# 1275468127/Medical-SAM2

Hardware: AMD Instinct MI355X
Metric: slices/sec @1024^2 (Hiera-S) (higher is better)
Workload: dtype bf16; 1 GPU; configs[1]: sam2_hiera_s 2D (train_2d SAM2 sub-sequence, forward), b=4 x 1024x1024 per GPU, 16-entry memory bank with 4 sampled memories per slice, one click per slice; forward_image -> memory_attention -> prompt encoder -> mask decoder -> memory encoder; hip_graph=True, weights=random name-keyed init

## Files before the change

### medical-sam2_amd/csrc/mlp_fused.hip

```cpp
#include "common.h"

struct MlpFusedParams {
  const float* x;
  float* out;
  const float *ln_w, *ln_b, *b1, *b2;
  const op16* w1;
  const op16* w2p;
  int64_t T;
  float eps;
  op16* out16;
};

template <int RB>
__device__ __forceinline__ int mlp_swz(int c, int r) {
  if constexpr (RB == 192) return (c & ~3) | ((c & 3) ^ ((r >> 2) & 3));
  else return (c & ~7) | ((c & 7) ^ ((r >> 1) & 7));
}

template <int DIM, int HC, int TB, int OCC = 1, int NWV = 4>
__global__ __launch_bounds__(NWV * 64, OCC) void mlp_fused_kernel(MlpFusedParams p) {
#if defined(__HIP_DEVICE_COMPILE__)
  constexpr int HID = 4 * DIM, NCH = HID / HC, KS1 = DIM / 16, DB = DIM / 32, HB = HC / 32;
  constexpr int RB1 = DIM * 2, RB2 = HC * 2;
  constexpr int CPR1 = DIM / 8, CPR2 = HC / 8;
  constexpr int W1B = HC * RB1, W2B = DIM * RB2, BUF = W1B + W2B;
  constexpr int PIECES1 = W1B / 1024, PIECES2 = W2B / 1024, PW1 = (PIECES1 + NWV - 1) / NWV, PW2 = (PIECES2 + NWV - 1) / NWV;
  static_assert((RB1 == 192 || RB1 == 384) && (RB2 == 192 || RB2 == 384), "row swizzles are built for 192 / 384-byte rows");
  static_assert(2 * BUF + (3 * DIM + HID) * 4 <= 160 * 1024, "LDS budget");
  extern __shared__ __attribute__((aligned(1024))) unsigned char smem[];
  float* prm = reinterpret_cast<float*>(smem + 2 * BUF);

  const int tid = threadIdx.x;
  const int wave = __builtin_amdgcn_readfirstlane(tid >> 6), lane = tid & 63;
  const int r = lane & 31, h = lane >> 5;
  for (int i = tid; i < DIM; i += NWV * 64) {
    prm[i] = p.ln_w[i];
    prm[DIM + i] = p.ln_b[i];
    prm[2 * DIM + i] = p.b2[i];
  }
  for (int i = tid; i < HID; i += NWV * 64) prm[3 * DIM + i] = p.b1[i];

  const auto w1_rsrc = raw_rsrc(p.w1, HID * DIM * 2);
  const auto w2_rsrc = raw_rsrc(p.w2p, HID * DIM * 2);
  unsigned off1[PW1], off2[PW2];
#pragma unroll
  for (int j = 0; j < PW1; ++j) {
    const int f = min(j * NWV + wave, PIECES1 - 1) * 64 + lane, row = f / CPR1, c = f % CPR1;
    off1[j] = (unsigned)(row * RB1 + mlp_swz<RB1>(c, row) * 16);
  }
#pragma unroll
  for (int j = 0; j < PW2; ++j) {
    const int f = min(j * NWV + wave, PIECES2 - 1) * 64 + lane, row = f / CPR2, c = f % CPR2;
    off2[j] = (unsigned)(row * HID * 2 + mlp_swz<RB2>(c, row) * 16);
  }
  auto issue = [&](int chunk, int buf) {
    unsigned char* d1 = smem + buf * BUF;
    unsigned char* d2 = smem + buf * BUF + W1B;
    const unsigned s1 = (unsigned)chunk * HC * RB1, s2 = (unsigned)chunk * HC * 2;
#pragma unroll
    for (int j = 0; j < PW1; ++j)
      if (j * NWV + wave < PIECES1)
        glds16(w1_rsrc, d1 + (j * NWV + wave) * 1024, off1[j], s1);
#pragma unroll
    for (int j = 0; j < PW2; ++j)
      if (j * NWV + wave < PIECES2)
        glds16(w2_rsrc, d2 + (j * NWV + wave) * 1024, off2[j], s2);
  };

  const int64_t pass_tokens = NWV * 32 * TB;
  const int64_t n_pass = (p.T + pass_tokens - 1) / pass_tokens;
  int64_t g_chunk = 0;
  constexpr bool RESIDENT = (NCH == 2) && NWV == 8;
  if ((int64_t)blockIdx.x < n_pass) {
    issue(0, 0);
    if constexpr (RESIDENT) issue(1, 1);
  }
  if constexpr (RESIDENT) wait_vmcnt<0>();
  __syncthreads();

  for (int64_t pass = blockIdx.x; pass < n_pass; pass += gridDim.x) {
    op16x8 xf[TB][KS1];
    int64_t tok[TB];
#pragma unroll
    for (int tb = 0; tb < TB; ++tb) {
      const int64_t t = pass * pass_tokens + (int64_t)(wave * TB + tb) * 32 + r;
      tok[tb] = t;
      const float* xr = p.x + (t < p.T ? t : p.T - 1) * DIM;
      f32x4 v[KS1][2];
      float s = 0.f;
#pragma unroll
      for (int k = 0; k < KS1; ++k)
#pragma unroll
        for (int q = 0; q < 2; ++q) {
          v[k][q] = *reinterpret_cast<const f32x4*>(xr + 16 * k + 8 * h + 4 * q);
          s += v[k][q][0] + v[k][q][1] + v[k][q][2] + v[k][q][3];
        }
      s += __shfl_xor(s, 32, 64);
      const float mean = s * (1.f / DIM);
      float q2 = 0.f;
#pragma unroll
      for (int k = 0; k < KS1; ++k)
#pragma unroll
        for (int q = 0; q < 2; ++q)
#pragma unroll
          for (int e = 0; e < 4; ++e) {
            const float dlt = v[k][q][e] - mean;
            q2 += dlt * dlt;
          }
      q2 += __shfl_xor(q2, 32, 64);
      const float rstd = 1.0f / sqrtf(q2 * (1.f / DIM) + p.eps);
#pragma unroll
      for (int k = 0; k < KS1; ++k) {
        op16x8 f;
#pragma unroll
        for (int q = 0; q < 2; ++q) {
          const f32x4 gm = *reinterpret_cast<const f32x4*>(prm + 16 * k + 8 * h + 4 * q);
          const f32x4 bt = *reinterpret_cast<const f32x4*>(prm + DIM + 16 * k + 8 * h + 4 * q);
#pragma unroll
          for (int e = 0; e < 4; ++e) f[4 * q + e] = f2op((v[k][q][e] - mean) * rstd * gm[e] + bt[e]);
        }
        xf[tb][k] = f;
      }
    }
    f32x16 accy[TB][DB];
#pragma unroll
    for (int tb = 0; tb < TB; ++tb)
#pragma unroll
      for (int d = 0; d < DB; ++d)
#pragma unroll
        for (int e = 0; e < 16; ++e) accy[tb][d][e] = 0.f;

    for (int chunk = 0; chunk < NCH; ++chunk, ++g_chunk) {
      const int buf = RESIDENT ? chunk : (int)(g_chunk & 1);
      if constexpr (!RESIDENT) {
        wait_vmcnt<0>();
        __builtin_amdgcn_s_barrier();
        const bool more_here = chunk + 1 < NCH;
        const bool more = more_here || (pass + gridDim.x < n_pass);
        if (more) issue(more_here ? chunk + 1 : 0, buf ^ 1);
      }
      const unsigned char* w1s = smem + buf * BUF;
      const unsigned char* w2s = w1s + W1B;
#pragma unroll 1
      for (int hb = 0; hb < HB; ++hb) {
        op16x8 a1[KS1];
        const int row1 = hb * 32 + r;
#pragma unroll
        for (int k = 0; k < KS1; ++k) a1[k] = *reinterpret_cast<const op16x8*>(w1s + row1 * RB1 + (mlp_swz<RB1>(2 * k + h, row1) << 4));
        f32x4 bias1[4];
#pragma unroll
        for (int g = 0; g < 4; ++g) bias1[g] = *reinterpret_cast<const f32x4*>(prm + 3 * DIM + chunk * HC + hb * 32 + 8 * g + 4 * h);
#pragma unroll
        for (int tb = 0; tb < TB; ++tb) {
          f32x16 acch;
#pragma unroll
          for (int e = 0; e < 16; ++e) acch[e] = bias1[e >> 2][e & 3];
#pragma unroll
          for (int k = 0; k < KS1; ++k) acch = MSAM2_MFMA_32x32x16(a1[k], xf[tb][k], acch, 0, 0, 0);
          op16x8 hf[2];
#pragma unroll
#ifdef MSAM2_MLP_NO_GELU
          for (int e = 0; e < 16; ++e) hf[e >> 3][e & 7] = f2op(acch[e]);
#else
          for (int e = 0; e < 16; e += 2) {
            const f32x2 gp = gelu_erf2(f32x2{acch[e], acch[e + 1]});
            hf[e >> 3][e & 7] = f2op(gp[0]);
            hf[e >> 3][(e & 7) + 1] = f2op(gp[1]);
          }
#endif
#pragma unroll
          for (int d = 0; d < DB; ++d) {
            const int row2 = d * 32 + r;
#pragma unroll
            for (int s2 = 0; s2 < 2; ++s2) {
              const op16x8 a2 = *reinterpret_cast<const op16x8*>(w2s + row2 * RB2 + (mlp_swz<RB2>(hb * 4 + 2 * s2 + h, row2) << 4));
              accy[tb][d] = MSAM2_MFMA_32x32x16(a2, hf[s2], accy[tb][d], 0, 0, 0);
            }
          }
        }
      }
    }
#pragma unroll
    for (int tb = 0; tb < TB; ++tb) {
      if (tok[tb] < p.T) {
        const float* xr = p.x + tok[tb] * DIM;
        float* yr = p.out + tok[tb] * DIM;
        constexpr int DG = 1;
        static_assert(DB % DG == 0, "d-blocks in whole batches");
#pragma unroll
        for (int d0 = 0; d0 < DB; d0 += DG) {
          f32x4 xv[DG][4];
#pragma unroll
          for (int d = 0; d < DG; ++d)
#pragma unroll
            for (int g = 0; g < 4; ++g) xv[d][g] = *reinterpret_cast<const f32x4*>(xr + (d0 + d) * 32 + 8 * g + 4 * h);
#pragma unroll
          for (int d = 0; d < DG; ++d)
#pragma unroll
            for (int g = 0; g < 4; ++g) {
              const int ch = (d0 + d) * 32 + 8 * g + 4 * h;
              const f32x4 bv = *reinterpret_cast<const f32x4*>(prm + 2 * DIM + ch);
              f32x4 o;
#pragma unroll
              for (int e = 0; e < 4; ++e) o[e] = accy[tb][d0 + d][4 * g + e] + bv[e] + xv[d][g][e];
              *reinterpret_cast<f32x4*>(yr + ch) = o;
              if (p.out16) {
                op16x4 o2;
#pragma unroll
                for (int e = 0; e < 4; ++e) o2[e] = f2op(o[e]);
                *reinterpret_cast<op16x4*>(p.out16 + tok[tb] * DIM + ch) = o2;
              }
            }
        }
      }
    }
  }
#endif
}

__device__ __forceinline__ int mlp_swz768(int c, int r) { return (c & ~15) | ((c & 15) ^ (r & 15)); }

__global__ __launch_bounds__(256, 1) void mlp_fused384_kernel(MlpFusedParams p) {
#if defined(__HIP_DEVICE_COMPILE__)
  constexpr int DIM = 384, HID = 1536, HC = 32, NCH = HID / HC, KS1 = DIM / 16, DBW = 6, NST = 3;
  constexpr int W1B = HC * DIM * 2, W2B = DIM * HC * 2, BUF = W1B + W2B;
  constexpr int PW = W1B / 1024 / 4;
  static_assert(NST * BUF + (3 * DIM + HID) * 4 <= 160 * 1024, "LDS budget");
  extern __shared__ __attribute__((aligned(1024))) unsigned char smem[];
  float* prm = reinterpret_cast<float*>(smem + NST * BUF);

  const int tid = threadIdx.x;
  const int wave = __builtin_amdgcn_readfirstlane(tid >> 6), lane = tid & 63;
  const int r = lane & 31, h = lane >> 5;
  const int tb = wave >> 1, dh = wave & 1;
  for (int i = tid; i < DIM; i += 256) {
    prm[i] = p.ln_w[i];
    prm[DIM + i] = p.ln_b[i];
    prm[2 * DIM + i] = p.b2[i];
  }
  for (int i = tid; i < HID; i += 256) prm[3 * DIM + i] = p.b1[i];

  const int64_t t = (int64_t)blockIdx.x * 64 + tb * 32 + r;
  const float* xr = p.x + (t < p.T ? t : p.T - 1) * DIM;
  f32x4 v[KS1][2];
#pragma unroll
  for (int k = 0; k < KS1; ++k)
#pragma unroll
    for (int q = 0; q < 2; ++q) v[k][q] = *reinterpret_cast<const f32x4*>(xr + 16 * k + 8 * h + 4 * q);

  const auto w1_rsrc = raw_rsrc(p.w1, HID * DIM * 2);
  const auto w2_rsrc = raw_rsrc(p.w2p, HID * DIM * 2);
  unsigned off1[PW];
#pragma unroll
  for (int j = 0; j < PW; ++j) {
    const int f = (j * 4 + wave) * 64 + lane, row = f / 48, c = f % 48;
    off1[j] = (unsigned)(row * 768 + mlp_swz768(c, row) * 16);
  }
  const unsigned off2 = (unsigned)(wave * 1024 + lane * 16);
  auto issue = [&](int i) {
    unsigned char* d1 = smem + (i % NST) * BUF;
    unsigned char* d2 = d1 + W1B;
    if (i < NCH) {
      const unsigned s = (unsigned)i * W1B;
#pragma unroll
      for (int j = 0; j < PW; ++j)
        glds16(w1_rsrc, d1 + (j * 4 + wave) * 1024, off1[j], s);
    }
    if (i >= 1) {
      const unsigned s = (unsigned)(i - 1) * W2B;
#pragma unroll
      for (int j = 0; j < PW; ++j)
        glds16(w2_rsrc, d2 + (j * 4 + wave) * 1024, off2, s + j * 4096);
    }
  };
  issue(0);
  issue(1);

  op16x8 xf[KS1];
  {
    float s = 0.f;
#pragma unroll
    for (int k = 0; k < KS1; ++k)
#pragma unroll
      for (int q = 0; q < 2; ++q) s += v[k][q][0] + v[k][q][1] + v[k][q][2] + v[k][q][3];
    s += __shfl_xor(s, 32, 64);
    const float mean = s * (1.f / DIM);
    float q2 = 0.f;
#pragma unroll
    for (int k = 0; k < KS1; ++k)
#pragma unroll
      for (int q = 0; q < 2; ++q)
#pragma unroll
        for (int e = 0; e < 4; ++e) {
          const float dlt = v[k][q][e] - mean;
          q2 += dlt * dlt;
        }
    q2 += __shfl_xor(q2, 32, 64);
    const float rstd = 1.0f / sqrtf(q2 * (1.f / DIM) + p.eps);
    __builtin_amdgcn_s_waitcnt(0xc07f);
    __builtin_amdgcn_s_barrier();
    asm volatile("" ::: "memory");
#pragma unroll
    for (int k = 0; k < KS1; ++k) {
      op16x8 f;
#pragma unroll
      for (int q = 0; q < 2; ++q) {
        const f32x4 gm = *reinterpret_cast<const f32x4*>(prm + 16 * k + 8 * h + 4 * q);
        const f32x4 bt = *reinterpret_cast<const f32x4*>(prm + DIM + 16 * k + 8 * h + 4 * q);
#pragma unroll
        for (int e = 0; e < 4; ++e) f[4 * q + e] = f2op((v[k][q][e] - mean) * rstd * gm[e] + bt[e]);
      }
      xf[k] = f;
    }
  }
  f32x16 accy[DBW];
#pragma unroll
  for (int d = 0; d < DBW; ++d)
#pragma unroll
    for (int e = 0; e < 16; ++e) accy[d][e] = 0.f;

  auto fc1_gelu = [&](const unsigned char* w1s, int chunk, f32x16& acch, const f32x16* aprev, op16x8 (&hf)[2]) {
    op16x8 fa[8], fb[8];
    auto rd = [&](op16x8 (&f)[8], int k0) {
#pragma unroll
      for (int k = 0; k < 8; ++k) f[k] = *reinterpret_cast<const op16x8*>(w1s + r * 768 + (mlp_swz768(2 * (k0 + k) + h, r) << 4));
    };
    rd(fa, 0);
    rd(fb, 8);
    f32x4 bias1[4];
#pragma unroll
    for (int g = 0; g < 4; ++g) bias1[g] = *reinterpret_cast<const f32x4*>(prm + 3 * DIM + chunk * HC + 8 * g + 4 * h);
    f32x16 part[2];
#pragma unroll
    for (int e = 0; e < 16; ++e) {
      part[0][e] = bias1[e >> 2][e & 3];
      part[1][e] = 0.f;
    }
    __builtin_amdgcn_sched_barrier(0);
#pragma unroll
    for (int k = 0; k < 8; ++k) part[k & 1] = MSAM2_MFMA_32x32x16(fa[k], xf[k], part[k & 1], 0, 0, 0);
    if (aprev) {
#pragma unroll
      for (int e = 0; e < 6; e += 2) {
        const f32x2 gp = gelu_erf2(f32x2{(*aprev)[e], (*aprev)[e + 1]});
        hf[e >> 3][e & 7] = f2op(gp[0]);
        hf[e >> 3][(e & 7) + 1] = f2op(gp[1]);
      }
    }
#pragma unroll
    for (int q = 0; q < 8; ++q) {
      __builtin_amdgcn_sched_group_barrier(0x008, 1, 0);
      __builtin_amdgcn_sched_group_barrier(0x002, 6, 0);
    }
    __builtin_amdgcn_sched_barrier(0);
    rd(fa, 16);
#pragma unroll
    for (int k = 0; k < 8; ++k) part[k & 1] = MSAM2_MFMA_32x32x16(fb[k], xf[8 + k], part[k & 1], 0, 0, 0);
    if (aprev) {
#pragma unroll
      for (int e = 6; e < 12; e += 2) {
        const f32x2 gp = gelu_erf2(f32x2{(*aprev)[e], (*aprev)[e + 1]});
        hf[e >> 3][e & 7] = f2op(gp[0]);
        hf[e >> 3][(e & 7) + 1] = f2op(gp[1]);
      }
    }
#pragma unroll
    for (int q = 0; q < 8; ++q) {
      __builtin_amdgcn_sched_group_barrier(0x008, 1, 1);
      __builtin_amdgcn_sched_group_barrier(0x002, 6, 1);
    }
    __builtin_amdgcn_sched_barrier(0);
#pragma unroll
    for (int k = 0; k < 8; ++k) part[k & 1] = MSAM2_MFMA_32x32x16(fa[k], xf[16 + k], part[k & 1], 0, 0, 0);
    if (aprev) {
#pragma unroll
      for (int e = 12; e < 16; e += 2) {
        const f32x2 gp = gelu_erf2(f32x2{(*aprev)[e], (*aprev)[e + 1]});
        hf[e >> 3][e & 7] = f2op(gp[0]);
        hf[e >> 3][(e & 7) + 1] = f2op(gp[1]);
      }
    }
#pragma unroll
    for (int q = 0; q < 8; ++q) {
      __builtin_amdgcn_sched_group_barrier(0x008, 1, 2);
      __builtin_amdgcn_sched_group_barrier(0x002, 5, 2);
    }
    __builtin_amdgcn_sched_barrier(0);
#pragma unroll
    for (int e = 0; e < 16; ++e) acch[e] = part[0][e] + part[1][e];
  };
  auto gelu16 = [&](const f32x16& acch, op16x8 (&hf)[2]) {
#pragma unroll
    for (int e = 0; e < 16; e += 2) {
      const f32x2 gp = gelu_erf2(f32x2{acch[e], acch[e + 1]});
      hf[e >> 3][e & 7] = f2op(gp[0]);
      hf[e >> 3][(e & 7) + 1] = f2op(gp[1]);
    }
  };
  auto fc2 = [&](const unsigned char* w2s, const op16x8 (&hf)[2]) {
    op16x8 a2[DBW][2];
#pragma unroll
    for (int d = 0; d < DBW; ++d) {
      const int row2 = (dh * DBW + d) * 32 + r;
#pragma unroll
      for (int s2 = 0; s2 < 2; ++s2) a2[d][s2] = *reinterpret_cast<const op16x8*>(w2s + row2 * Img64::ROW_BYTES + (((2 * s2 + h) ^ Img64::swz(row2)) << 4));
    }
#pragma unroll
    for (int s2 = 0; s2 < 2; ++s2)
#pragma unroll
      for (int d = 0; d < DBW; ++d) accy[d] = MSAM2_MFMA_32x32x16(a2[d][s2], hf[s2], accy[d], 0, 0, 0);
  };

  f32x16 acur;
  wait_vmcnt<12>();
  __builtin_amdgcn_s_barrier();
  issue(2);
  {
    op16x8 hf0[2];
    fc1_gelu(smem, 0, acur, nullptr, hf0);
  }
#pragma unroll 1
  for (int i = 1; i < NCH; ++i) {
    if (i + 1 < NCH) wait_vmcnt<12>();
    else wait_vmcnt<6>();
    __builtin_amdgcn_s_barrier();
    if (i + 2 <= NCH) issue(i + 2);
    const unsigned char* w1s = smem + (i % NST) * BUF;
    f32x16 anext;
    op16x8 hf[2];
    fc1_gelu(w1s, i, anext, &acur, hf);
    fc2(w1s + W1B, hf);
    acur = anext;
  }
  {
    wait_vmcnt<0>();
    __builtin_amdgcn_s_barrier();
    op16x8 hf[2];
    gelu16(acur, hf);
    fc2(smem + (NCH % NST) * BUF + W1B, hf);
  }

  if (t < p.T) {
    const float* xres = p.x + t * DIM;
    float* yr = p.out + t * DIM;
    constexpr int DG = 3;
#pragma unroll
    for (int d0 = 0; d0 < DBW; d0 += DG) {
      f32x4 xv[DG][4];
#pragma unroll
      for (int d = 0; d < DG; ++d)
#pragma unroll
        for (int g = 0; g < 4; ++g) xv[d][g] = *reinterpret_cast<const f32x4*>(xres + (dh * DBW + d0 + d) * 32 + 8 * g + 4 * h);
#pragma unroll
      for (int d = 0; d < DG; ++d)
#pragma unroll
        for (int g = 0; g < 4; ++g) {
          const int ch = (dh * DBW + d0 + d) * 32 + 8 * g + 4 * h;
          const f32x4 bv = *reinterpret_cast<const f32x4*>(prm + 2 * DIM + ch);
          f32x4 o;
#pragma unroll
          for (int e = 0; e < 4; ++e) o[e] = accy[d0 + d][4 * g + e] + bv[e] + xv[d][g][e];
          *reinterpret_cast<f32x4*>(yr + ch) = o;
          if (p.out16) {
            op16x4 o2;
#pragma unroll
            for (int e = 0; e < 4; ++e) o2[e] = f2op(o[e]);
            *reinterpret_cast<op16x4*>(p.out16 + t * DIM + ch) = o2;
          }
        }
    }
  }
#endif
}

__global__ void mlp_fused384_pack_kernel(const op16* __restrict__ w2, op16* __restrict__ w2q, int dim, int hid) {
  const int64_t total = (int64_t)dim * hid;
  for (int64_t i = (int64_t)blockIdx.x * blockDim.x + threadIdx.x; i < total; i += (int64_t)gridDim.x * blockDim.x) {
    const int chunk = (int)(i / ((int64_t)dim * 32)), d = (int)((i / 32) % dim), q = (int)(i & 31);
    const int c = (q >> 3) ^ Img64::swz(d), j = q & 7, pos = c * 8 + j;
    const int s = pos >> 4, hh = (pos >> 3) & 1;
    w2q[i] = w2[(int64_t)d * hid + chunk * 32 + 16 * s + 8 * (j >> 2) + 4 * hh + (j & 3)];
  }
}

__global__ void mlp_fused_permute_kernel(const op16* __restrict__ w2, op16* __restrict__ w2p, int dim, int hid) {
  const int64_t total = (int64_t)dim * hid;
  for (int64_t i = (int64_t)blockIdx.x * blockDim.x + threadIdx.x; i < total; i += (int64_t)gridDim.x * blockDim.x) {
    const int d = (int)(i / hid), pos = (int)(i % hid);
    const int blk = pos >> 5, q = pos & 31, s = q >> 4, hh = (q >> 3) & 1, j = q & 7;
    w2p[i] = w2[(int64_t)d * hid + blk * 32 + 16 * s + 8 * (j >> 2) + 4 * hh + (j & 3)];
  }
}

extern "C" int msam2_mlp_fused_permute_w2(const void* w2, void* w2p, int64_t dim, int64_t hidden, void* stream) {
  MSAM2_REQUIRE(w2 && w2p && dim > 0 && hidden % 32 == 0, "mlp_fused_permute_w2: bad arguments");
  if (dim == 384) {
    MSAM2_REQUIRE(hidden == 1536, "mlp_fused_permute_w2: dim 384 takes hidden 1536");
    hipLaunchKernelGGL(mlp_fused384_pack_kernel, dim3(1024), dim3(256), 0, (hipStream_t)stream, (const op16*)w2, (op16*)w2p, (int)dim, (int)hidden);
    return msam2_check_launch("mlp_fused_permute_w2(384)");
  }
  hipLaunchKernelGGL(mlp_fused_permute_kernel, dim3((unsigned)min((int64_t)1024, cdiv(dim * hidden, 256))), dim3(256), 0, (hipStream_t)stream,
                     (const op16*)w2, (op16*)w2p, (int)dim, (int)hidden);
  return msam2_check_launch("mlp_fused_permute_w2");
}

extern "C" int msam2_ln_mlp_residual_supported(int64_t dim) {
  static const bool use384 = [] { const char* e = getenv("MSAM2_MLP_384"); return e && e[0] == '1'; }();
  return dim == 96 || dim == 192 || (dim == 384 && use384);
}

static int launch_mlp_fused384(const MlpFusedParams& p, hipStream_t s) {
  constexpr int LDS = 3 * 49152 + (3 * 384 + 1536) * 4;
  ensure_dyn_lds<mlp_fused384_kernel>(LDS);
  hipLaunchKernelGGL(mlp_fused384_kernel, dim3((unsigned)((p.T + 63) / 64)), dim3(256), LDS, s, p);
  return msam2_check_launch("ln_mlp_residual_fwd(384)");
}

template <int DIM, int HC, int TB, int OCC = 1, int NWV = 4>
static int launch_mlp_fused(const MlpFusedParams& p, hipStream_t s) {
  constexpr int LDS = 2 * (2 * HC * DIM * 2) + (3 * DIM + 4 * DIM) * 4;
  ensure_dyn_lds<mlp_fused_kernel<DIM, HC, TB, OCC, NWV>>(LDS);
  const int64_t n_pass = (p.T + NWV * 32 * TB - 1) / (NWV * 32 * TB);
  hipLaunchKernelGGL((mlp_fused_kernel<DIM, HC, TB, OCC, NWV>), dim3((unsigned)min((int64_t)256 * OCC, n_pass)), dim3(NWV * 64), LDS, s, p);
  return msam2_check_launch("ln_mlp_residual_fwd");
}

static int ln_mlp_residual_launch(const float* x, int64_t T, int64_t dim, const float* ln_w, const float* ln_b, float eps, const void* w1,
                                  const float* b1, const void* w2p, const float* b2, float* out, void* out16, void* stream) {
  MSAM2_REQUIRE(x && out && ln_w && ln_b && w1 && b1 && w2p && b2 && T > 0, "ln_mlp_residual: null tensor / empty problem");
  MSAM2_REQUIRE(dim == 96 || dim == 192 || dim == 384, "ln_mlp_residual: dim %lld not built (96 / 192 / 384)", (long long)dim);
  MSAM2_REQUIRE((((uintptr_t)x | (uintptr_t)out | (uintptr_t)w1 | (uintptr_t)w2p | (uintptr_t)ln_w | (uintptr_t)ln_b | (uintptr_t)b1 | (uintptr_t)b2) & 15) == 0 &&
                    ((uintptr_t)out16 & 7) == 0, "ln_mlp_residual: 16-byte aligned tensors");
  MSAM2_REQUIRE(x != out, "ln_mlp_residual: in-place not supported (a token's residual is re-read in the store)");
  MlpFusedParams p = {x, out, ln_w, ln_b, b1, b2, (const op16*)w1, (const op16*)w2p, T, eps, (op16*)out16};
  hipStream_t s = (hipStream_t)stream;
  if (dim == 384) {
    MSAM2_REQUIRE((T + 63) / 64 < (1ll << 31), "ln_mlp_residual: too many tokens");
    return launch_mlp_fused384(p, s);
  }
  static const bool four = [] { const char* e = getenv("MSAM2_MLP_WAVES4"); return e && e[0] == '1'; }();
  if (four) {
    if (dim == 96) return launch_mlp_fused<96, 192, 4>(p, s);
    return launch_mlp_fused<192, 96, 2>(p, s);
  }
  if (dim == 96) return launch_mlp_fused<96, 192, 2, 1, 8>(p, s);
  return launch_mlp_fused<192, 96, 1, 1, 8>(p, s);
}

extern "C" int msam2_ln_mlp_residual_fwd(const float* x, int64_t T, int64_t dim, const float* ln_w, const float* ln_b, float eps, const void* w1,
                                         const float* b1, const void* w2p, const float* b2, float* out, void* stream) {
  return ln_mlp_residual_launch(x, T, dim, ln_w, ln_b, eps, w1, b1, w2p, b2, out, nullptr, stream);
}

extern "C" int msam2_ln_mlp_residual_fwd_dual(const float* x, int64_t T, int64_t dim, const float* ln_w, const float* ln_b, float eps,
                                              const void* w1, const float* b1, const void* w2p, const float* b2, float* out, void* out16,
                                              void* stream) {
  MSAM2_REQUIRE(out16, "ln_mlp_residual_dual: null 16-bit output");
  return ln_mlp_residual_launch(x, T, dim, ln_w, ln_b, eps, w1, b1, w2p, b2, out, out16, stream);
}
```

### medical-sam2_amd/ops.py

```python
from __future__ import annotations

import ctypes
import math
from typing import Optional, Tuple

import torch

from ._lib import check, lib

OP16 = torch.float16 if lib().msam2_operand_is_fp16() else torch.bfloat16

F32 = torch.float32
ACT_NONE, ACT_GELU, ACT_RELU, ACT_SIGMOID = 0, 1, 2, 3


def _stream() -> int:
    return torch.cuda.current_stream().cuda_stream


def _p(t: Optional[torch.Tensor]):
    return None if t is None else t.data_ptr()


def _is_bf16(t: torch.Tensor) -> int:
    if t.dtype == OP16:
        return 1
    if t.dtype == F32:
        return 0
    raise TypeError(f"expected {OP16} or fp32 tensor, got {t.dtype}")


def _req(cond: bool, msg: str):
    if not cond:
        raise ValueError(msg)


def gemm(a: torch.Tensor, w: torch.Tensor, bias: Optional[torch.Tensor] = None, *, act: int = ACT_NONE,
         colscale: Optional[torch.Tensor] = None, residual: Optional[torch.Tensor] = None, res_mod: int = 0,
         out_dtype: torch.dtype = OP16, out: Optional[torch.Tensor] = None) -> torch.Tensor:
    _req(a.dim() == 2 and w.dim() == 2 and a.shape[1] == w.shape[1], f"gemm shapes {tuple(a.shape)} x {tuple(w.shape)}")
    _req(a.dtype == OP16 and w.dtype == OP16, "gemm operands must be 16-bit (ops.OP16)")
    _req(a.stride(1) == 1 and w.stride(1) == 1, "gemm operands must be K-contiguous")
    M, K = a.shape
    N = w.shape[0]
    if out is None:
        out = torch.empty(M, N, dtype=out_dtype, device=a.device)
    _req(out.stride(1) == 1 and out.shape == (M, N), "gemm out must be [M,N] row-major")
    if residual is not None:
        _req(residual.dim() == 2 and residual.stride(1) == 1 and residual.shape[1] == N, "gemm residual must be [*,N]")
    check(lib().msam2_gemm(_p(a), a.stride(0), _p(w), w.stride(0), _p(bias), _p(colscale), _p(residual),
                                residual.stride(0) if residual is not None else 0,
                                _is_bf16(residual) if residual is not None else 0, res_mod, _p(out), out.stride(0),
                                _is_bf16(out), M, N, K, act, _stream()))
    return out


def gemm_tokens(a: torch.Tensor, w: torch.Tensor, bias: Optional[torch.Tensor] = None, *, addend: Optional[torch.Tensor] = None,
                add_cols: int = 0, act: int = ACT_NONE, residual: Optional[torch.Tensor] = None, out_dtype: torch.dtype = OP16) -> torch.Tensor:
    _req(a.dim() == 2 and a.dtype == F32 and a.stride(1) == 1 and a.shape[0] <= 32, "gemm_tokens: a must be fp32 [M<=32, K]")
    _req(w.dtype == OP16 and w.stride(1) == 1 and w.shape[1] == a.shape[1], "gemm_tokens: w must be 16-bit [N, K]")
    if addend is not None:
        _req(addend.dtype == F32 and addend.shape == a.shape and addend.stride(1) == 1 and addend.stride(0) == a.stride(0),
             "gemm_tokens: addend must match a")
    M, K = a.shape
    N = w.shape[0]
    out = torch.empty(M, N, dtype=out_dtype, device=a.device)
    if residual is not None:
        _req(residual.dtype == F32 and residual.shape == (M, N) and residual.stride(1) == 1, "gemm_tokens: residual must be fp32 [M,N]")
    check(lib().msam2_gemm_tokens(_p(a), a.stride(0), _p(addend), add_cols if addend is not None else 0, _p(w), w.stride(0), _p(bias),
                                  _p(residual), residual.stride(0) if residual is not None else 0, _p(out), out.stride(0), _is_bf16(out),
                                  M, N, K, act, _stream()))
    return out


def gemm_pool2x2(a: torch.Tensor, w: torch.Tensor, bias: Optional[torch.Tensor], B: int, H: int, W: int) -> torch.Tensor:
    _req(a.dim() == 2 and w.dim() == 2 and a.shape[1] == w.shape[1] and a.shape[0] == B * H * W, "gemm_pool2x2 shapes")
    _req(a.dtype == OP16 and w.dtype == OP16 and a.stride(1) == 1 and w.stride(1) == 1, "gemm_pool2x2 operands: 16-bit, K-contiguous")
    N, K = w.shape
    out = torch.empty(B * (H // 2) * (W // 2), N, dtype=F32, device=a.device)
    check(lib().msam2_gemm_pool2x2(_p(a), a.stride(0), _p(w), w.stride(0), _p(bias), _p(out), out.stride(0), B, H, W, N, K, _stream()))
    return out


def gemm_qkv_pool2x2(a: torch.Tensor, w: torch.Tensor, bias: Optional[torch.Tensor], B: int, H: int, W: int, q_cols: int):
    _req(a.dim() == 2 and w.dim() == 2 and a.shape[1] == w.shape[1] and a.shape[0] == B * H * W, "gemm_qkv_pool2x2 shapes")
    _req(a.dtype == OP16 and w.dtype == OP16 and a.stride(1) == 1 and w.stride(1) == 1, "gemm_qkv_pool2x2 operands: 16-bit, K-contiguous")
    N, K = w.shape
    qkv = torch.empty(B * H * W, N, dtype=OP16, device=a.device)
    q2 = torch.empty(B * (H // 2) * (W // 2), q_cols, dtype=OP16, device=a.device)
    check(lib().msam2_gemm_qkv_pool2x2(_p(a), a.stride(0), _p(w), w.stride(0), _p(bias), _p(qkv), qkv.stride(0), _p(q2), q2.stride(0),
                                       B, H, W, N, K, q_cols, _stream()))
    return qkv, q2


def gemm_rope(a: torch.Tensor, w: torch.Tensor, bias: Optional[torch.Tensor], table: Tuple[torch.Tensor, torch.Tensor], *,
              rope_cols: int, head_dim: int, rows_per_batch: int, n_rope: int, out: Optional[torch.Tensor] = None) -> torch.Tensor:
    _req(a.dim() == 2 and w.dim() == 2 and a.shape[1] == w.shape[1], f"gemm_rope shapes {tuple(a.shape)} x {tuple(w.shape)}")
    _req(a.dtype == OP16 and w.dtype == OP16 and a.stride(1) == 1 and w.stride(1) == 1, "gemm_rope operands: 16-bit, K-contiguous")
    cs, sn = table
    _req(cs.dtype == F32 and cs.is_contiguous() and sn.is_contiguous() and cs.shape == sn.shape and cs.shape[1] * 2 == head_dim,
         "gemm_rope: table must be cos/sin fp32 [n_pos, head_dim/2]")
    M, K = a.shape
    N = w.shape[0]
    if out is None:
        out = torch.empty(M, N, dtype=OP16, device=a.device)
    _req(out.dtype == OP16 and out.shape == (M, N) and out.stride(1) == 1, "gemm_rope: out must be 16-bit [M, N] row-major")
    check(lib().msam2_gemm_rope(_p(a), a.stride(0), _p(w), w.stride(0), _p(bias), _p(out), out.stride(0), M, N, K, _p(cs), _p(sn),
                                rope_cols, head_dim, rows_per_batch, n_rope, cs.shape[0], _stream()))
    return out


def layernorm(x: torch.Tensor, weight: torch.Tensor, bias: torch.Tensor, eps: float, *, act: int = ACT_NONE,
              out_dtype: torch.dtype = OP16) -> torch.Tensor:
    C = x.shape[-1]
    x2 = x.reshape(-1, C)
    _req(x2.stride(1) == 1, "layernorm input rows must be contiguous")
    y = torch.empty(x2.shape, dtype=out_dtype, device=x.device)
    check(lib().msam2_layernorm(_p(x2), _is_bf16(x2), x2.stride(0), _p(weight), _p(bias), _p(y), _is_bf16(y), y.stride(0),
                                x2.shape[0], C, eps, act, _stream()))
    return y.reshape(x.shape)


def layernorm_dual(x: torch.Tensor, weight: torch.Tensor, bias: torch.Tensor, eps: float):
    C = x.shape[-1]
    x2 = x.reshape(-1, C)
    _req(x2.dtype == F32 and x2.stride(1) == 1 and C % 4 == 0, "layernorm_dual: fp32 rows, C % 4 == 0")
    y = torch.empty(x2.shape, dtype=F32, device=x.device)
    y16 = torch.empty(x2.shape, dtype=OP16, device=x.device)
    check(lib().msam2_layernorm_dual(_p(x2), x2.stride(0), _p(weight), _p(bias), _p(y), y.stride(0), _p(y16), y16.stride(0), x2.shape[0], C, eps,
                                     _stream()))
    return y.reshape(x.shape), y16.reshape(x.shape)


def ln_mlp_residual_supported(dim: int) -> bool:
    return bool(lib().msam2_ln_mlp_residual_supported(dim))


def mlp_fused_permute_w2(w2: torch.Tensor) -> torch.Tensor:
    _req(w2.dim() == 2 and w2.dtype == OP16 and w2.is_contiguous() and w2.shape[1] % 32 == 0, "mlp_fused_permute_w2: 16-bit [dim, hidden]")
    out = torch.empty_like(w2)
    check(lib().msam2_mlp_fused_permute_w2(_p(w2), _p(out), w2.shape[0], w2.shape[1], _stream()))
    return out


def ln_mlp_residual(x: torch.Tensor, ln_w: torch.Tensor, ln_b: torch.Tensor, eps: float, w1: torch.Tensor, b1: torch.Tensor, w2p: torch.Tensor,
                    b2: torch.Tensor, also16: bool = False):
    T, dim = x.shape
    _req(x.dtype == F32 and x.is_contiguous() and w1.dtype == OP16 and w2p.dtype == OP16 and w1.shape == (4 * dim, dim) and w2p.shape == (dim, 4 * dim)
         and w1.is_contiguous() and w2p.is_contiguous(), "ln_mlp_residual: x fp32 [T, dim], w1 [4 dim, dim], w2p [dim, 4 dim] 16-bit contiguous")
    out = torch.empty_like(x)
    if also16:
        out16 = torch.empty(x.shape, dtype=OP16, device=x.device)
        check(lib().msam2_ln_mlp_residual_fwd_dual(_p(x), T, dim, _p(ln_w), _p(ln_b), float(eps), _p(w1), _p(b1), _p(w2p), _p(b2), _p(out), _p(out16),
                                                   _stream()))
        return out, out16
    check(lib().msam2_ln_mlp_residual_fwd(_p(x), T, dim, _p(ln_w), _p(ln_b), float(eps), _p(w1), _p(b1), _p(w2p), _p(b2), _p(out), _stream()))
    return out


def _strides3(t: torch.Tensor) -> "ctypes.Array":
    return (ctypes.c_int64 * 3)(t.stride(0), t.stride(1), t.stride(2))


def attention(q: torch.Tensor, k: torch.Tensor, v: torch.Tensor, *, splits: int = 1,
              out: Optional[torch.Tensor] = None, scale: Optional[float] = None, workspace: Optional[torch.Tensor] = None,
              defer_merge: bool = False, lse: Optional[torch.Tensor] = None, dropout: Optional[tuple] = None) -> torch.Tensor:
    B, H, Lq, D = q.shape
    Lk = k.shape[2]
    for t in (q, k, v):
        _req(t.dtype == OP16 and t.stride(3) == 1, "attention tensors must be 16-bit (ops.OP16) with contiguous head dim")
    if out is None:
        out = torch.empty(B, Lq, H, D, dtype=OP16, device=q.device).permute(0, 2, 1, 3)
    if lse is not None:
        _req(lse.dtype == F32 and lse.is_contiguous() and lse.numel() == B * H * Lq and not defer_merge, "attention: lse must be fp32 [B,H,Lq]")
        splits = max(splits, 2)
    ws_bytes = lib().msam2_attention_workspace_bytes(B, H, Lq, D, splits)
    ws = workspace if workspace is not None else (torch.empty(max(ws_bytes, 1), dtype=torch.uint8, device=q.device) if splits > 1 else None)
    _req(not defer_merge or (workspace is not None and splits > 1), "defer_merge needs splits > 1 and a caller-owned workspace")
    _req(ws is None or ws.numel() * ws.element_size() >= ws_bytes, "attention workspace too small")
    sc = scale if scale is not None else 1.0 / math.sqrt(D)
    if dropout is not None and dropout[0] > 0:
        _req(lse is not None, "attention: dropout is a training feature (pass lse)")
        pd, seed, offset = dropout
        seed_dev = None
        if isinstance(seed, DeviceSeed):
            seed, seed_dev = seed.base, seed.dev
        check(lib().msam2_attention_fwd_lse_dropout(_p(q), _strides3(q), _p(k), _strides3(k), _p(v), _strides3(v), _p(out), _strides3(out),
                                                    B, H, Lq, Lk, D, sc, splits, _p(ws), ws_bytes if ws is not None else 0, _p(lse), float(pd),
                                                    int(seed) & (2 ** 64 - 1), int(offset) & (2 ** 64 - 1), _p(seed_dev), _stream()))
        return out
    if lse is not None:
        check(lib().msam2_attention_fwd_lse(_p(q), _strides3(q), _p(k), _strides3(k), _p(v), _strides3(v), _p(out), _strides3(out),
                                            B, H, Lq, Lk, D, sc, splits, _p(ws), ws_bytes if ws is not None else 0, _p(lse), _stream()))
        return out
    check(lib().msam2_attention_fwd(_p(q), _strides3(q), _p(k), _strides3(k), _p(v), _strides3(v), _p(out), _strides3(out),
                                    B, H, Lq, Lk, D, sc, -splits if defer_merge else splits, _p(ws), ws_bytes if ws is not None else 0, _stream()))
    return out


def attention_kv64(q: torch.Tensor, k: torch.Tensor, v: torch.Tensor, *, splits: int = 1, scale: Optional[float] = None,
                   workspace: Optional[torch.Tensor] = None, defer_merge: bool = False,
                   key_count: Optional[torch.Tensor] = None, out: Optional[torch.Tensor] = None) -> torch.Tensor:
    B, H, Lq, D = q.shape
    Lk = k.shape[2]
    _req(D == 256 and k.shape[3] == 256 and v.shape[3] == 64 and v.shape[2] == Lk, "attention_kv64: q/k rows of 256, v rows of 64")
    _req(key_count is None or (key_count.dtype == torch.int32 and key_count.numel() == 1 and key_count.device == q.device),
         "attention_kv64: key_count is one int32 on the tensors' device")
    for t in (q, k, v):
        _req(t.dtype == OP16 and t.stride(3) == 1, "attention tensors must be 16-bit (ops.OP16) with contiguous head dim")
    if out is None:
        out = torch.empty(B, Lq, H, 64, dtype=OP16, device=q.device).permute(0, 2, 1, 3)
    _req(out.dtype == OP16 and out.shape == (B, H, Lq, 64) and out.stride(3) == 1, "attention_kv64: out is a 16-bit [B,H,Lq,64] view")
    ws_bytes = lib().msam2_attention_workspace_bytes(B, H, Lq, 64, splits)
    ws = workspace if workspace is not None else (torch.empty(max(ws_bytes, 1), dtype=torch.uint8, device=q.device) if splits > 1 else None)
    _req(not defer_merge or (workspace is not None and splits > 1), "defer_merge needs splits > 1 and a caller-owned workspace")
    _req(ws is None or ws.numel() * ws.element_size() >= ws_bytes, "attention workspace too small")
    sc = scale if scale is not None else 1.0 / math.sqrt(D)
    if key_count is not None:
        check(lib().msam2_attention_kv64_dyn_fwd(_p(q), _strides3(q), _p(k), _strides3(k), _p(v), _strides3(v), _p(out), _strides3(out),
                                                 B, H, Lq, Lk, _p(key_count), sc, -splits if defer_merge else splits, _p(ws),
                                                 ws_bytes if ws is not None else 0, _stream()))
        return out
    check(lib().msam2_attention_kv64_fwd(_p(q), _strides3(q), _p(k), _strides3(k), _p(v), _strides3(v), _p(out), _strides3(out),
                                         B, H, Lq, Lk, sc, -splits if defer_merge else splits, _p(ws), ws_bytes if ws is not None else 0, _stream()))
    return out


def attention_effective_splits(Lk: int, splits: int) -> int:
    return int(lib().msam2_attention_effective_splits(Lk, splits))


def attention_kv64_partial(q: torch.Tensor, k: torch.Tensor, v: torch.Tensor, *, splits: int, split_begin: int, split_count: int,
                           workspace: torch.Tensor, scale: Optional[float] = None, key_count: Optional[torch.Tensor] = None) -> None:
    B, H, Lq, D = q.shape
    Lk = k.shape[2]
    for t in (q, k, v):
        _req(t.dtype == OP16 and t.stride(3) == 1, "attention tensors must be 16-bit (ops.OP16) with contiguous head dim")
    sc = scale if scale is not None else 1.0 / math.sqrt(D)
    if key_count is not None:
        _req(key_count.dtype == torch.int32 and key_count.numel() == 1, "attention_kv64_partial: key_count is one int32 on the device")
        check(lib().msam2_attention_kv64_dyn_partial(_p(q), _strides3(q), _p(k), _strides3(k), _p(v), _strides3(v), B, H, Lq, Lk, _p(key_count),
                                                     sc, splits, split_begin, split_count, _p(workspace),
                                                     workspace.numel() * workspace.element_size(), _stream()))
        return
    check(lib().msam2_attention_kv64_partial(_p(q), _strides3(q), _p(k), _strides3(k), _p(v), _strides3(v), B, H, Lq, Lk, sc, splits,
                                             split_begin, split_count, _p(workspace), workspace.numel() * workspace.element_size(), _stream()))


def attention_workspace(B: int, H: int, Lq: int, D: int, splits: int, device) -> torch.Tensor:
    return torch.empty(max(lib().msam2_attention_workspace_bytes(B, H, Lq, D, splits), 1), dtype=torch.uint8, device=device)


def attention_merge(out: torch.Tensor, Lk: int, splits: int, workspace: torch.Tensor) -> torch.Tensor:
    B, H, Lq, D = out.shape
    check(lib().msam2_attention_merge(_p(out), _strides3(out), B, H, Lq, Lk, D, splits, _p(workspace),
                                      workspace.numel() * workspace.element_size(), _stream()))
    return out


def window_attention(qkv: torch.Tensor, B: int, H: int, W: int, heads: int, ws: int, qkv_bias: torch.Tensor,
                     q_pooled: Optional[torch.Tensor] = None, scale: Optional[float] = None,
                     out: Optional[torch.Tensor] = None) -> torch.Tensor:
    dim_out = qkv.shape[1] // 3
    D = dim_out // heads
    _req(qkv.dtype == OP16 and qkv.stride(1) == 1, "qkv must be 16-bit (ops.OP16) row-major")
    if q_pooled is None:
        qt, q_ts, hq, wq, ws_q = qkv, qkv.stride(0), H, W, ws
    else:
        qt, q_ts, hq, wq, ws_q = q_pooled, q_pooled.stride(0), H // 2, W // 2, ws // 2
    o = out if out is not None else torch.empty(B * hq * wq, dim_out, dtype=OP16, device=qkv.device)
    _req(o.dtype == OP16 and o.shape == (B * hq * wq, dim_out) and o.stride(1) == 1, "window_attention: out is 16-bit [B*Hq*Wq, heads*D] rows")
    kpad = qkv_bias[dim_out:2 * dim_out]
    vpad = qkv_bias[2 * dim_out:]
    kptr = qkv.data_ptr() + dim_out * 2
    vptr = qkv.data_ptr() + 2 * dim_out * 2
    check(lib().msam2_window_attention_fwd(_p(qt), q_ts, D, hq, wq, ws_q, kptr, vptr, qkv.stride(0), D, H, W, ws, _p(kpad),
                                           _p(vpad), _p(o), o.stride(0), D, B, heads, D, scale if scale is not None else 1.0 / math.sqrt(D), _stream()))
    return o


def attention_small(q: torch.Tensor, k: torch.Tensor, v: torch.Tensor, heads: int, out: Optional[torch.Tensor] = None) -> torch.Tensor:
    B, Lq, C = q.shape
    Lk = k.shape[1]
    D = C // heads
    for t in (q, k, v):
        _req(t.dtype == OP16 and t.stride(2) == 1, "attention_small tensors must be 16-bit (ops.OP16), channel-contiguous")
    o = out if out is not None else torch.empty(B, Lq, C, dtype=OP16, device=q.device)
    _req(o.dtype == OP16 and o.shape == (B, Lq, C) and o.stride(2) == 1, "attention_small: out is 16-bit [B,Lq,C] with contiguous channels")
    check(lib().msam2_attention_small_fwd(_p(q), q.stride(0), q.stride(1), _p(k), k.stride(0), k.stride(1), _p(v), v.stride(0),
                                          v.stride(1), _p(o), o.stride(0), o.stride(1), B, heads, Lq, Lk, D,
                                          1.0 / math.sqrt(D), _stream()))
    return o


def add_cast(a: torch.Tensor, b: Optional[torch.Tensor] = None, alpha: float = 1.0, out_dtype: torch.dtype = OP16,
             out: Optional[torch.Tensor] = None) -> torch.Tensor:
    _req(a.dim() == 3 and (a.stride(2) == 1 or a.shape[2] == 1), "add_cast: a must be [D0,D1,C] with contiguous C")
    D0, D1, C = a.shape
    bs0 = bs1 = 0
    if b is not None:
        b = b.expand(D0, D1, C)
        _req(b.stride(2) == 1 or C == 1, "add_cast: b must have contiguous C")
        bs0, bs1 = b.stride(0), b.stride(1)
    if out is None:
        out = torch.empty(D0, D1, C, dtype=out_dtype, device=a.device)
    _req(out.is_contiguous() and out.numel() == D0 * D1 * C, "add_cast: out must be a contiguous [D0,D1,C] buffer")
    check(lib().msam2_add_cast(_p(a), _is_bf16(a), a.stride(0), a.stride(1), _p(b), _is_bf16(b) if b is not None else 0, bs0,
                               bs1, alpha, _p(out), _is_bf16(out), D0, D1, C, _stream()))
    return out


class DeviceSeed:
    __slots__ = ("base", "dev")

    def __init__(self, base: int, dev: torch.Tensor):
        assert dev.dtype == torch.int64 and dev.numel() == 1 and dev.is_cuda
        self.base, self.dev = int(base), dev


def counter_bump(counter: torch.Tensor, snapshot: Optional[torch.Tensor] = None) -> None:
    _req(counter.dtype == torch.int64 and counter.numel() == 1 and (snapshot is None or (snapshot.dtype == torch.int64 and snapshot.numel() == 1)),
         "counter_bump: int64 [1] tensors")
    check(lib().msam2_counter_bump(_p(counter), _p(snapshot), _stream()))


def dropout(x: torch.Tensor, p: float, seed, offset: int, residual: Optional[torch.Tensor] = None,
            out_dtype: Optional[torch.dtype] = None, out: Optional[torch.Tensor] = None) -> torch.Tensor:
    seed_dev = None
    if isinstance(seed, DeviceSeed):
        seed, seed_dev = seed.base, seed.dev
    _req(x.dim() == 2 and x.stride(1) == 1, "dropout: [rows, cols] row-major")
    rows, cols = x.shape
    y = out if out is not None else torch.empty(rows, cols, dtype=out_dtype or x.dtype, device=x.device)
    _req(y.shape == x.shape and y.stride(1) == 1, "dropout: out must be [rows, cols] row-major (rows may be strided)")
    if residual is not None:
        _req(residual.dtype == F32 and residual.shape == x.shape and residual.stride(1) == 1, "dropout: residual must be fp32 [rows, cols]")
    check(lib().msam2_dropout(_p(x), _is_bf16(x), x.stride(0), _p(residual), residual.stride(0) if residual is not None else 0, _p(y), _is_bf16(y),
                              y.stride(0), rows, cols, float(p), int(seed) & (2 ** 64 - 1), int(offset) & (2 ** 64 - 1), _p(seed_dev), _stream()))
    return y


def add_cast_into(out: torch.Tensor, a: torch.Tensor, b: Optional[torch.Tensor] = None, alpha: float = 1.0) -> torch.Tensor:
    return add_cast(a, b, alpha, out=out)


def gate_no_obj_(x: torch.Tensor, score: torch.Tensor, value: float) -> torch.Tensor:
    _req(x.dtype == F32 and x.is_contiguous(), "gate_no_obj: fp32 contiguous")
    B = x.shape[0]
    check(lib().msam2_gate_rows(_p(x), _p(score), value, B, x.numel() // B, _stream()))
    return x


def any_positive(x: torch.Tensor) -> torch.Tensor:
    _req(x.dtype == F32 and x.is_contiguous(), "any_positive: fp32 contiguous")
    B = x.shape[0]
    out = torch.empty(B, 1, dtype=F32, device=x.device)
    check(lib().msam2_any_positive(_p(x), _p(out), B, x.numel() // B, _stream()))
    return out


def maxpool2x2(x: torch.Tensor, B: int, H: int, W: int, out_dtype: Optional[torch.dtype] = None) -> torch.Tensor:
    C = x.shape[1]
    _req(x.stride(1) == 1, "maxpool2x2: channel dim must be contiguous")
    y = torch.empty(B * (H // 2) * (W // 2), C, dtype=out_dtype or x.dtype, device=x.device)
    check(lib().msam2_maxpool2x2(_p(x), _is_bf16(x), x.stride(0), _p(y), _is_bf16(y), y.stride(0), B, H, W, C, _stream()))
    return y


def upsample2x_add_(y: torch.Tensor, top: torch.Tensor, B: int, H: int, W: int) -> torch.Tensor:
    _req(y.dtype == F32 and top.dtype == F32 and y.is_contiguous() and top.is_contiguous(), "upsample2x_add: fp32 contiguous")
    check(lib().msam2_upsample2x_add(_p(y), _p(top), B, H, W, y.shape[-1], _stream()))
    return y


def rope_table(side: int, D: int, theta: float, device) -> Tuple[torch.Tensor, torch.Tensor]:
    cs = torch.empty(side * side, D // 2, dtype=F32, device=device)
    sn = torch.empty_like(cs)
    check(lib().msam2_rope_table(_p(cs), _p(sn), side, D, theta, _stream()))
    return cs, sn


def rope_(x: torch.Tensor, n_rope: int, table: Tuple[torch.Tensor, torch.Tensor]) -> torch.Tensor:
    B, L, D = x.shape
    _req(x.dtype == OP16 and x.stride(2) == 1, "rope: 16-bit with contiguous D")
    cs, sn = table
    check(lib().msam2_rope_inplace(_p(x), x.stride(0), x.stride(1), B, L, n_rope, cs.shape[0], D, _p(cs), _p(sn), _stream()))
    return x


def bilinear_upsample(x: torch.Tensor, H: int, W: int) -> torch.Tensor:
    _req(x.dtype == F32 and x.is_contiguous(), "bilinear: fp32 contiguous")
    h, w = x.shape[-2:]
    planes = x.numel() // (h * w)
    y = torch.empty(*x.shape[:-2], H, W, dtype=F32, device=x.device)
    check(lib().msam2_bilinear_upsample(_p(x), _p(y), planes, h, w, H, W, _stream()))
    return y


def sine_pos_2d(h: int, w: int, C: int, device, temperature: float = 10000.0) -> torch.Tensor:
    out = torch.empty(h * w, C, dtype=F32, device=device)
    check(lib().msam2_sine_pos_2d(_p(out), h, w, C, temperature, _stream()))
    return out


def fourier_pe_grid(gauss: torch.Tensor, h: int, w: int) -> torch.Tensor:
    C = 2 * gauss.shape[1]
    out = torch.empty(h * w, C, dtype=F32, device=gauss.device)
    check(lib().msam2_fourier_pe_grid(_p(out), _p(gauss.contiguous()), h, w, C, _stream()))
    return out


def hiera_pos_embed(pos_embed: torch.Tensor, pos_embed_window: torch.Tensor, h: int, w: int) -> torch.Tensor:
    _, C, bh, bw = pos_embed.shape
    out = torch.empty(h * w, C, dtype=F32, device=pos_embed.device)
    check(lib().msam2_hiera_pos_embed(_p(out), _p(pos_embed.contiguous()), _p(pos_embed_window.contiguous()), C, bh, bw, h, w,
                                      pos_embed_window.shape[-1], _stream()))
    return out


def im2col_patch(img: torch.Tensor) -> torch.Tensor:
    _req(img.dtype == F32 and img.is_contiguous() and img.shape[1] == 3 and img.shape[2] == img.shape[3], "im2col_patch: [B,3,S,S] fp32")
    B, _, S, _ = img.shape
    out = torch.empty(B * (S // 4) ** 2, 160, dtype=OP16, device=img.device)
    check(lib().msam2_im2col_patch7x7s4(_p(img), _p(out), B, S, _stream()))
    return out


def patch_embed_supported(S: int, E: int) -> bool:
    So = S // 4
    return S % 4 == 0 and So % 32 == 0 and E <= 128


def patch_embed(img: torch.Tensor, w_perm: torch.Tensor, bias: torch.Tensor, pos: Optional[torch.Tensor] = None) -> torch.Tensor:
    _req(img.dtype == F32 and img.is_contiguous() and img.shape[1] == 3 and img.shape[2] == img.shape[3], "patch_embed: [B,3,S,S] fp32")
    B, _, S, _ = img.shape
    E = bias.shape[0]
    _req(patch_embed_supported(S, E), "patch_embed: unsupported size (use im2col_patch + gemm)")
    _req(w_perm.dtype == OP16 and w_perm.is_contiguous() and tuple(w_perm.shape) == ((E + 31) // 32 * 32, 176), "patch_embed: w_perm [ceil32(E), 176] 16-bit")
    _req(bias.dtype == F32 and bias.is_contiguous(), "patch_embed: fp32 bias")
    if pos is not None:
        _req(pos.dtype == F32 and pos.is_contiguous() and tuple(pos.shape) == ((S // 4) ** 2, E), "patch_embed: pos fp32 [(S/4)^2, E]")
    out = torch.empty(B * (S // 4) ** 2, E, dtype=F32, device=img.device)
    check(lib().msam2_patch_embed7x7s4(_p(img), _p(w_perm), _p(bias), _p(pos), _p(out), B, S, E, _stream()))
    return out


def im2col3x3s2(x: torch.Tensor, B: int, H: int, W: int) -> torch.Tensor:
    C = x.shape[-1]
    _req(x.dtype == OP16 and x.is_contiguous(), "im2col3x3s2: 16-bit contiguous NHWC")
    ld = (9 * C + 7) // 8 * 8
    out = torch.empty(B * (H // 2) * (W // 2), ld, dtype=OP16, device=x.device)
    check(lib().msam2_im2col3x3s2(_p(x), _p(out), B, H, W, C, ld, _stream()))
    return out


# ... 714 lines not shown
```

Measured before the change: 686.7 slices/s.

## Add LDS-staged x/output path to fused MLP and default dim-96 to TB=1

New measurement: 689.7 slices/s (median of 6 runs). No clear change (+0.4%).

```diff
diff --git a/medical-sam2_amd/csrc/mlp_fused.hip b/medical-sam2_amd/csrc/mlp_fused.hip
--- a/medical-sam2_amd/csrc/mlp_fused.hip
+++ b/medical-sam2_amd/csrc/mlp_fused.hip
@@ -12,12 +12,49 @@
 };
 
 template <int RB>
-__device__ __forceinline__ int mlp_swz(int c, int r) {
+__host__ __device__ constexpr int mlp_swz(int c, int r) {
   if constexpr (RB == 192) return (c & ~3) | ((c & 3) ^ ((r >> 2) & 3));
   else return (c & ~7) | ((c & 7) ^ ((r >> 1) & 7));
 }
-
-template <int DIM, int HC, int TB, int OCC = 1, int NWV = 4>
+__host__ __device__ constexpr int mlp_swz768(int c, int r) { return (c & ~15) | ((c & 15) ^ (r & 15)); }
+
+template <int XRB>
+__host__ __device__ constexpr int mlp_xswz(int c, int r) {
+  static_assert(XRB == 384 || XRB == 768, "x-row images exist for dim 96 / 192");
+  if constexpr (XRB == 384) return mlp_swz<384>(c, r);
+  else return mlp_swz768(c, r);
+}
+template <int RB, typename F>
+constexpr bool mlp_image_ok(F swz) {
+  constexpr int CPR = RB / 16;
+  for (int r = 0; r < 32; ++r) {
+    unsigned long long seen = 0;
+    for (int c = 0; c < CPR; ++c) {
+      const int s = swz(c, r);
+      if (s < 0 || s >= CPR || ((seen >> s) & 1)) return false;
+      seen |= 1ull << s;
+    }
+  }
+  for (int c = 0; c < CPR; ++c)
+    for (int grp = 0; grp < 2; ++grp) {
+      unsigned banks = 0;
+      for (int r = 0; r < 32; ++r) {
+        const bool first = r < 4 || (r >= 12 && r < 16) || (r >= 20 && r < 28);
+        if (first != (grp == 0)) continue;
+        const int bg = ((r * RB + swz(c, r) * 16) / 16) & 15;
+        if ((banks >> bg) & 1) return false;
+        banks |= 1u << bg;
+      }
+      if (banks != 0xffffu) return false;
+    }
+  return true;
+}
+static_assert(mlp_image_ok<192>([](int c, int r) { return mlp_swz<192>(c, r); }), "192-byte weight rows");
+static_assert(mlp_image_ok<384>([](int c, int r) { return mlp_swz<384>(c, r); }), "384-byte weight rows / dim-96 x rows");
+static_assert(mlp_image_ok<128>([](int c, int r) { return mlp_swz<128>(c, r); }), "128-byte weight rows");
+static_assert(mlp_image_ok<768>([](int c, int r) { return mlp_swz768(c, r); }), "768-byte weight rows / dim-192 x rows");
+
+template <int DIM, int HC, int TB, int OCC = 1, int NWV = 4, bool STG = false>
 __global__ __launch_bounds__(NWV * 64, OCC) void mlp_fused_kernel(MlpFusedParams p) {
 #if defined(__HIP_DEVICE_COMPILE__)
   constexpr int HID = 4 * DIM, NCH = HID / HC, KS1 = DIM / 16, DB = DIM / 32, HB = HC / 32;
@@ -25,10 +62,11 @@
   constexpr int CPR1 = DIM / 8, CPR2 = HC / 8;
   constexpr int W1B = HC * RB1, W2B = DIM * RB2, BUF = W1B + W2B;
   constexpr int PIECES1 = W1B / 1024, PIECES2 = W2B / 1024, PW1 = (PIECES1 + NWV - 1) / NWV, PW2 = (PIECES2 + NWV - 1) / NWV;
-  static_assert((RB1 == 192 || RB1 == 384) && (RB2 == 192 || RB2 == 384), "row swizzles are built for 192 / 384-byte rows");
-  static_assert(2 * BUF + (3 * DIM + HID) * 4 <= 160 * 1024, "LDS budget");
+  static_assert((RB1 == 192 || RB1 == 384) && (RB2 == 128 || RB2 == 192 || RB2 == 384), "row swizzles are built for 128 / 192 / 384-byte rows");
+  constexpr int XRB = DIM * 4, XCPR = DIM / 4, SLAB = 32 * XRB, XP = SLAB / 1024, STGB = STG ? NWV * SLAB : 0;
+  static_assert(2 * BUF + STGB + (3 * DIM + HID) * 4 <= 160 * 1024, "LDS budget");
   extern __shared__ __attribute__((aligned(1024))) unsigned char smem[];
-  float* prm = reinterpret_cast<float*>(smem + 2 * BUF);
+  float* prm = reinterpret_cast<float*>(smem + 2 * BUF + STGB);
 
   const int tid = threadIdx.x;
   const int wave = __builtin_amdgcn_readfirstlane(tid >> 6), lane = tid & 63;
@@ -69,6 +107,19 @@
 
   const int64_t pass_tokens = NWV * 32 * TB;
   const int64_t n_pass = (p.T + pass_tokens - 1) / pass_tokens;
+  [[maybe_unused]] unsigned char* slab = smem + 2 * BUF + (STG ? wave * SLAB : 0);
+  [[maybe_unused]] auto stage_in = [&](int64_t t0) {
+    const int64_t left = p.T - t0;
+    const int rows = left >= 32 ? 32 : (left > 0 ? (int)left : 0);
+    const auto x_rsrc = raw_rsrc(p.x + (rows ? t0 : 0) * DIM, rows * XRB);
+    asm volatile("s_waitcnt lgkmcnt(0)" ::: "memory");
+#pragma unroll
+    for (int j = 0; j < XP; ++j) {
+      const int f = j * 64 + lane, row = f / XCPR, c = f % XCPR;
+      glds16(x_rsrc, slab + j * 1024, (unsigned)(row * XRB + mlp_xswz<XRB>(c, row) * 16), 0);
+    }
+    wait_vmcnt<0>();
+  };
   int64_t g_chunk = 0;
   constexpr bool RESIDENT = (NCH == 2) && NWV == 8;
   if ((int64_t)blockIdx.x < n_pass) {
@@ -86,13 +137,15 @@
       const int64_t t = pass * pass_tokens + (int64_t)(wave * TB + tb) * 32 + r;
       tok[tb] = t;
       const float* xr = p.x + (t < p.T ? t : p.T - 1) * DIM;
+      if constexpr (STG) stage_in(pass * pass_tokens + (int64_t)(wave * TB + tb) * 32);
       f32x4 v[KS1][2];
       float s = 0.f;
 #pragma unroll
       for (int k = 0; k < KS1; ++k)
 #pragma unroll
         for (int q = 0; q < 2; ++q) {
-          v[k][q] = *reinterpret_cast<const f32x4*>(xr + 16 * k + 8 * h + 4 * q);
+          if constexpr (STG) v[k][q] = *reinterpret_cast<const f32x4*>(slab + r * XRB + (mlp_xswz<XRB>(4 * k + 2 * h + q, r) << 4));
+          else v[k][q] = *reinterpret_cast<const f32x4*>(xr + 16 * k + 8 * h + 4 * q);
           s += v[k][q][0] + v[k][q][1] + v[k][q][2] + v[k][q][3];
         }
       s += __shfl_xor(s, 32, 64);
@@ -180,8 +233,51 @@
         }
       }
     }
-#pragma unroll
-    for (int tb = 0; tb < TB; ++tb) {
+    if constexpr (STG) {
+#pragma unroll
+      for (int tbi = 0; tbi < TB; ++tbi) {
+        const int tb = TB - 1 - tbi;
+        const int64_t t0 = pass * pass_tokens + (int64_t)(wave * TB + tb) * 32;
+        if (t0 >= p.T) continue;
+        if (tbi) stage_in(t0);
+#pragma unroll
+        for (int d = 0; d < DB; ++d)
+#pragma unroll
+          for (int g = 0; g < 4; ++g) {
+            f32x4* cell = reinterpret_cast<f32x4*>(slab + r * XRB + (mlp_xswz<XRB>(8 * d + 2 * g + h, r) << 4));
+            const f32x4 xv = *cell;
+            const f32x4 bv = *reinterpret_cast<const f32x4*>(prm + 2 * DIM + d * 32 + 8 * g + 4 * h);
+            f32x4 o;
+#pragma unroll
+            for (int e = 0; e < 4; ++e) o[e] = accy[tb][d][4 * g + e] + bv[e] + xv[e];
+            *cell = o;
+          }
+        asm volatile("s_waitcnt lgkmcnt(0)" ::: "memory");
+#pragma unroll
+        for (int j = 0; j < XP; ++j) {
+          const int f = j * 64 + lane, row = f / XCPR, c = f % XCPR;
+          const f32x4 o = *reinterpret_cast<const f32x4*>(slab + f * 16);
+          if (t0 + row < p.T) *reinterpret_cast<f32x4*>(p.out + (t0 + row) * DIM + mlp_xswz<XRB>(c, row) * 4) = o;
+        }
+        if (p.out16) {
+#pragma unroll
+          for (int j = 0; j < XP / 2; ++j) {
+            const int f = j * 64 + lane, row = f / (XCPR / 2), m = f % (XCPR / 2);
+            const f32x4 a = *reinterpret_cast<const f32x4*>(slab + row * XRB + (mlp_xswz<XRB>(2 * m, row) << 4));
+            const f32x4 b = *reinterpret_cast<const f32x4*>(slab + row * XRB + (mlp_xswz<XRB>(2 * m + 1, row) << 4));
+            op16x8 o2;
+#pragma unroll
+            for (int e = 0; e < 4; ++e) {
+              o2[e] = f2op(a[e]);
+              o2[4 + e] = f2op(b[e]);
+            }
+            if (t0 + row < p.T) *reinterpret_cast<op16x8*>(p.out16 + (t0 + row) * DIM + 8 * m) = o2;
+          }
+        }
+      }
+    }
+#pragma unroll
+    for (int tb = 0; tb < (STG ? 0 : TB); ++tb) {
       if (tok[tb] < p.T) {
         const float* xr = p.x + tok[tb] * DIM;
         float* yr = p.out + tok[tb] * DIM;
@@ -217,8 +313,6 @@
   }
 #endif
 }
-
-__device__ __forceinline__ int mlp_swz768(int c, int r) { return (c & ~15) | ((c & 15) ^ (r & 15)); }
 
 __global__ __launch_bounds__(256, 1) void mlp_fused384_kernel(MlpFusedParams p) {
 #if defined(__HIP_DEVICE_COMPILE__)
@@ -516,13 +610,22 @@
   return msam2_check_launch("ln_mlp_residual_fwd(384)");
 }
 
-template <int DIM, int HC, int TB, int OCC = 1, int NWV = 4>
+template <int DIM, int HC, int TB, int OCC = 1, int NWV = 4, bool STG = false>
 static int launch_mlp_fused(const MlpFusedParams& p, hipStream_t s) {
-  constexpr int LDS = 2 * (2 * HC * DIM * 2) + (3 * DIM + 4 * DIM) * 4;
-  ensure_dyn_lds<mlp_fused_kernel<DIM, HC, TB, OCC, NWV>>(LDS);
+  constexpr int LDS = 2 * (2 * HC * DIM * 2) + (STG ? NWV * 32 * DIM * 4 : 0) + (3 * DIM + 4 * DIM) * 4;
+  ensure_dyn_lds<mlp_fused_kernel<DIM, HC, TB, OCC, NWV, STG>>(LDS);
   const int64_t n_pass = (p.T + NWV * 32 * TB - 1) / (NWV * 32 * TB);
-  hipLaunchKernelGGL((mlp_fused_kernel<DIM, HC, TB, OCC, NWV>), dim3((unsigned)min((int64_t)256 * OCC, n_pass)), dim3(NWV * 64), LDS, s, p);
+  hipLaunchKernelGGL((mlp_fused_kernel<DIM, HC, TB, OCC, NWV, STG>), dim3((unsigned)min((int64_t)256 * OCC, n_pass)), dim3(NWV * 64), LDS, s, p);
   return msam2_check_launch("ln_mlp_residual_fwd");
+}
+
+static constexpr bool kMlpStagedDefault96 = false;
+static bool mlp_io_staged(int64_t dim) {
+  if (dim != 96) return false;
+  const char* e = getenv("MSAM2_MLP_IO");
+  if (e && e[0] == 'l') return 0;
+  if (e && e[0] == 's') return 1;
+  return kMlpStagedDefault96;
 }
 
 static int ln_mlp_residual_launch(const float* x, int64_t T, int64_t dim, const float* ln_w, const float* ln_b, float eps, const void* w1,
@@ -543,7 +646,12 @@
     if (dim == 96) return launch_mlp_fused<96, 192, 4>(p, s);
     return launch_mlp_fused<192, 96, 2>(p, s);
   }
-  if (dim == 96) return launch_mlp_fused<96, 192, 2, 1, 8>(p, s);
+  if (dim == 96) {
+    if (mlp_io_staged(96) && ((uintptr_t)out16 & 15) == 0) return launch_mlp_fused<96, 64, 1, 1, 8, true>(p, s);
+    const char* e = getenv("MSAM2_MLP_TB2");
+    if (e && e[0] == '1') return launch_mlp_fused<96, 192, 2, 1, 8>(p, s);
+    return launch_mlp_fused<96, 192, 1, 1, 8>(p, s);
+  }
   return launch_mlp_fused<192, 96, 1, 1, 8>(p, s);
 }
 
diff --git a/medical-sam2_amd/ops.py b/medical-sam2_amd/ops.py
--- a/medical-sam2_amd/ops.py
+++ b/medical-sam2_amd/ops.py
@@ -144,13 +144,16 @@
 
 
 def ln_mlp_residual(x: torch.Tensor, ln_w: torch.Tensor, ln_b: torch.Tensor, eps: float, w1: torch.Tensor, b1: torch.Tensor, w2p: torch.Tensor,
-                    b2: torch.Tensor, also16: bool = False):
+                    b2: torch.Tensor, also16: bool = False, out: torch.Tensor = None, out16: torch.Tensor = None):
     T, dim = x.shape
     _req(x.dtype == F32 and x.is_contiguous() and w1.dtype == OP16 and w2p.dtype == OP16 and w1.shape == (4 * dim, dim) and w2p.shape == (dim, 4 * dim)
          and w1.is_contiguous() and w2p.is_contiguous(), "ln_mlp_residual: x fp32 [T, dim], w1 [4 dim, dim], w2p [dim, 4 dim] 16-bit contiguous")
-    out = torch.empty_like(x)
+    for o, dt in ((out, F32), (out16, OP16)):
+        _req(o is None or (o.dtype == dt and o.dim() == 2 and o.shape[0] >= T and o.shape[1] == dim and o.is_contiguous() and o.device == x.device),
+             "ln_mlp_residual: out / out16 contiguous [>= T, dim] in fp32 / the 16-bit type")
+    out = torch.empty_like(x) if out is None else out[:T]
     if also16:
-        out16 = torch.empty(x.shape, dtype=OP16, device=x.device)
+        out16 = torch.empty(x.shape, dtype=OP16, device=x.device) if out16 is None else out16[:T]
         check(lib().msam2_ln_mlp_residual_fwd_dual(_p(x), T, dim, _p(ln_w), _p(ln_b), float(eps), _p(w1), _p(b1), _p(w2p), _p(b2), _p(out), _p(out16),
                                                    _stream()))
         return out, out16
```
